# m-dayani/EORB_SLAM

Hardware: AMD Instinct MI355X
Metric: front-end frames/s (event-accumulate + extract + match) per GPU; HBM GB/s vs roofline (higher is better)
Workload: dtype f32; 1 GPU; BASELINE.json configs[1]: synthetic 1000000 events/slice on 240x180 (shapes generator, DAVIS sensor pixels; raw (x,y,t,p) records resolved on the GPU through the calibrator's undistortion maps built from the EvETHZ intrinsics, as the reference loader does on the CPU), ev2im_gauss sigma=1 -> ORB-1000 (1.2, 4 levels, FAST 10/0, edge 19) -> SearchForInitialization vs previous slice; input=raw, sequences_per_gpu=1, parallelism=1 GPU

## Files before the change

### eorb_slam_amd/csrc/ev_common.h

```cpp
#pragma once
#include <hip/hip_runtime.h>
#include <stdint.h>
#include <string.h>
#include <algorithm>
#include <vector>
#include "eorb_ctx.h"

namespace eorb {

struct BinLayout {
    int B, nchunks, NT, nb;
    size_t cd, sc, eb, cnt;
    const ChunkDesc* d_chunks = nullptr; const int* d_slice_c0 = nullptr; const int64_t* d_slice_eb = nullptr;
    uint16_t* d_segcnt = nullptr; uint32_t* d_segbase = nullptr; uint32_t* d_tile_cnt = nullptr; uint32_t* d_tile_base = nullptr;
    BinLayout() : BinLayout(0, 0, 0) {}
    BinLayout(int B_, int nchunks_, int NT_) : B(B_), nchunks(nchunks_), NT(NT_), nb(B_ * NT_)
    {
        cd = sizeof(ChunkDesc) * (size_t)std::max(nchunks, 1);
        sc = (sizeof(int) * (size_t)(B + 1) + 7) & ~(size_t)7;
        eb = sizeof(int64_t) * (size_t)B;
        cnt = (sizeof(uint16_t) * (size_t)std::max(nchunks, 1) * NT + 15) & ~(size_t)15;
    }
    size_t chunks_bytes() const { return cd + sc + eb; }
    size_t segoff_bytes() const { return cnt + sizeof(uint32_t) * (size_t)std::max(nchunks, 1) * NT; }
    void view(void* chunks, void* segoff, void* tile_order)
    {
        d_chunks = (const ChunkDesc*)chunks; d_slice_c0 = (const int*)((char*)chunks + cd); d_slice_eb = (const int64_t*)((char*)chunks + cd + sc);
        d_segcnt = (uint16_t*)segoff; d_segbase = (uint32_t*)((char*)segoff + cnt);
        d_tile_cnt = (uint32_t*)tile_order; d_tile_base = d_tile_cnt + nb;
    }
};

struct EntryBaseRule { int per_event; int64_t slack; int64_t align; };
struct HostBins { std::vector<ChunkDesc> cds; std::vector<int> slice_c0; std::vector<int64_t> slice_eb; int64_t nchunks = 0, entries = 0; };

static inline HostBins bin_chunks_host(const int64_t* h_offsets, int B, int chunk, const EntryBaseRule& R, bool lists = true)
{
    HostBins hb;
    if (lists) { hb.slice_c0.resize(B + 1); hb.slice_eb.resize(B); }
    for (int b = 0; b < B; b++) {
        const int64_t s = h_offsets[b], e = h_offsets[b + 1];
        if (lists) {
            hb.slice_c0[b] = (int)hb.nchunks; hb.slice_eb[b] = hb.entries;
            for (int64_t k = s; k < e; k += chunk) {
                ChunkDesc cd; cd.start = k; cd.n = (int32_t)std::min<int64_t>(chunk, e - k); cd.slice = b;
// ... 63 lines not shown
```

### eorb_slam_amd/csrc/ev_plan.h

```cpp
#pragma once
#include <math.h>
#include <stddef.h>
#include <stdint.h>
#include <algorithm>

namespace eorb {

constexpr int kTile = 8;
constexpr int kChunk = 4096;
constexpr int kScatWaves = 8;
constexpr int kSlotScatWaves = 8;
constexpr int kSlotCountWaves = 16;
constexpr int kHotCap = 8192;
constexpr int kHotRows = 240;
constexpr int kDdLog = 20;
constexpr int kDirectSlices = 8;
constexpr int64_t kDirectMaxEvents = 16384;

struct AccumShape {
    int h;
    int R, dup;
    int TX, TY, NT, NTp;
    int nbits;
    int64_t nev, per_slice;
// ... 90 lines not shown
inline bool plan_sparse_gather(const AccumShape& S, const AccumRequest& Q, const AccumKnobs& K)
{
    return Q.raw && !Q.mode_count && (K.gather_form == 2 || (K.gather_form == 0 && plan_sparse_load(S, Q.B)));
}

enum { kGatherSparse, kGatherRawRows, kGatherGeneric };
struct GatherPlan { int kind, NC, threads, per_wave; };
inline GatherPlan plan_gather(const AccumShape& S, const AccumRequest& Q, const AccumKnobs& K)
{
    const int nb = Q.B * S.NT;
    if (plan_sparse_gather(S, Q, K)) return GatherPlan{kGatherSparse, 0, 0, nb >= 65536 ? 16 : 1};
    if (Q.raw && !Q.mode_count) {
        const int NC = K.gather_nc == 2 || K.gather_nc == 4 ? K.gather_nc : (nb >= 32768 ? 4 : 2);
        return GatherPlan{kGatherRawRows, NC, 64 * (1 + 8 / NC), 0};
    }
    return GatherPlan{kGatherGeneric, 0, K.gather_threads, 0};
}

struct SlotScatterChoice { int chunk, waves; bool rank; size_t lds; };
inline size_t plan_slot_lds_rank(int NT, int chunk, int waves) { const int NTp = (NT + 1) & ~1; return ((size_t)NT * 4 + (size_t)chunk * 4 * 2 + (size_t)waves * NTp * 2 + (size_t)(NTp + 2) * 2 + (size_t)chunk * 4 + 15) & ~(size_t)15; }
inline size_t plan_slot_lds_pre(int NT, int chunk) { const int NTp = (NT + 1) & ~1; return ((size_t)NT * 4 + (size_t)chunk * 4 * 2 + (size_t)(NTp + 2) * 2 + (size_t)chunk * 4 + 15) & ~(size_t)15; }
inline size_t plan_slot_lds_ballot(int NT, int chunk) { const int NTp = (NT + 1) & ~1; return ((size_t)chunk * 4 + (size_t)chunk * 2 + (size_t)chunk * 4 * 2 + (size_t)kSlotScatWaves * NTp * 2 + (size_t)(NTp + 2) * 2 + (size_t)NT * 4 + 15) & ~(size_t)15; }

inline bool plan_slot_scatter(const AccumShape& S, const AccumKnobs& K, bool rank_ok, SlotScatterChoice* out)
{
    const int pref = K.slot_chunk ? K.slot_chunk : (S.per_slice >= (int64_t)1 << 18 ? 4096 : (S.per_slice >= (int64_t)1 << 17 ? 2048 : (S.per_slice >= (int64_t)1 << 14 ? 1024 : 256)));
    const bool rank_allowed = rank_ok && K.slot_rank;
    static const int sizes[4] = {4096, 2048, 1024, 256};
    for (int i = 0; i < 4; i++) {
        const int chunk = sizes[i];
        if (chunk > pref) continue;
        if (rank_allowed) {
            const int waves = chunk == 4096 ? 16 : kSlotScatWaves;
            const size_t l = plan_slot_lds_rank(S.NT, chunk, waves);
            if (l <= (size_t)(chunk == 4096 ? 79 : 158) * 1024) { *out = SlotScatterChoice{chunk, waves, true, l}; return true; }
        }
        if (chunk <= 2048) {
            const size_t l = plan_slot_lds_ballot(S.NT, chunk);
            if (l <= 64 * 1024) { *out = SlotScatterChoice{chunk, kSlotScatWaves, false, l}; return true; }
        }
    }
    return false;
}

inline bool plan_slot_shape(const AccumShape& S, int B, const AccumKnobs& K, bool rank_ok, SlotScatterChoice* out)
{
    return !(B > 2048 || (size_t)S.NT * 4 > 64 * 1024 || !plan_slot_scatter(S, K, rank_ok, out));
}

enum { kCountGlobal, kCountLds, kCountLdsKeyed };
enum { kRecAsIs, kRecShort2, kRecRanked8 };
// ... 73 lines not shown
```

### eorb_slam_amd/csrc/ev_slots.hip

```cpp
#include "eorb_ctx.h"
#include "ev_common.h"
#include "dev_math.h"
#include "sl_hot_asm.h"
#include <algorithm>
#include <stdlib.h>
#include <string.h>
#include <vector>

namespace eorb {

constexpr uint32_t kNoSlot = 0xffu;
typedef uint16_t slot_entry;
constexpr uint32_t kEntryTag = 0x1000u;
constexpr uint16_t kNoGeo = 0xffffu;

__global__ void sl_assign_kernel(const uint32_t* __restrict__ src_info, int nsrc, int W, int H, int h, int TX,
                                 uint32_t* __restrict__ tile_nslots, uint2* __restrict__ slot_tab, uint16_t* __restrict__ slot_geo,
                                 int* __restrict__ info)
{
    const int i = blockIdx.x * blockDim.x + threadIdx.x;
    if (i >= nsrc) { if (i == nsrc) slot_geo[i] = kNoGeo; return; }
    const uint32_t w = src_info[i];
    const int xi = (int)(int16_t)(w & 0xffff), yi = (int)(int16_t)(w >> 16);
    uint2 o = make_uint2(0u, 0xffffffffu);
// ... 106 lines not shown
    }
    if (blockIdx.x == 0) {
        if (tid < B) slice_eb[tid] = e0[tid];
        for (int b = tid; b <= B; b += blockDim.x) slice_c0[b] = c0[b];
    }
    const int g = blockIdx.x * blockDim.x + tid;
    if (g >= nchunks) return;
    int lo = 0, hi = B;
    while (hi - lo > 1) { const int mid = (lo + hi) >> 1; if (c0[mid] <= g) lo = mid; else hi = mid; }
    const int64_t start = off[lo] + ((int64_t)(g - c0[lo]) << chunk_shift);
    ChunkDesc cd; cd.start = start; cd.n = (int32_t)min(chunk, off[lo + 1] - start); cd.slice = lo;
    chunks[g] = cd;
}

template <int stride>
__device__ __forceinline__ uint32_t sl_load_rec(const unsigned char* e, int k)
{
    if (stride == 2) { const uint32_t v = *(const uint16_t*)(e + (size_t)k * 2); return v == 0xffffu ? 0x7fffffffu : v; }
    return *(const uint32_t*)(e + (size_t)k * (size_t)(stride < 0 ? -stride : stride));
}
template <int stride>
__global__ __launch_bounds__(256) void sl_count_kernel(const eorb_raw_event* __restrict__ ev, const ChunkDesc* __restrict__ chunks,
                                                       const uint2* __restrict__ slot_tab, int LW, int LH, int TX, int NT,
                                                       uint16_t* __restrict__ segcnt)
{
    extern __shared__ uint32_t cnt[];
    const ChunkDesc cd = chunks[blockIdx.x];
    for (int i = threadIdx.x; i < NT; i += blockDim.x) cnt[i] = 0;
    __syncthreads();
    const unsigned char* e = (const unsigned char*)ev + (size_t)cd.start * (size_t)(stride < 0 ? -stride : stride);
    const uint32_t xmask = stride == 4 ? 0x7fffu : 0xffffu;
    const bool hashed = stride < 0 || stride == 2;
    constexpr int U = 8;
    for (int k0 = threadIdx.x; k0 < cd.n; k0 += blockDim.x * U) {
        uint32_t xy[U], rg[U];
#pragma unroll
        for (int u = 0; u < U; u++) { const int k = k0 + u * blockDim.x; xy[u] = k < cd.n ? sl_load_rec<stride>(e, k) : 0xffffffffu; }
#pragma unroll
        for (int u = 0; u < U; u++) {
            const int x = (int)(xy[u] & xmask), y = (int)(xy[u] >> 16);
            const uint32_t row = xy[u] & 0x7fffffffu;
            if (hashed) rg[u] = (row != 0x7fffffffu && row < (uint32_t)LW * (uint32_t)LH) ? slot_tab[row].x : 0u;
            else rg[u] = (x < LW && y < LH) ? slot_tab[(uint32_t)y * (uint32_t)LW + x].x : 0u;
        }
#pragma unroll
        for (int u = 0; u < U; u++) {
            const int nx = (rg[u] >> 16) & 3, ny = (rg[u] >> 18) & 3;
            const int t0 = (int)((rg[u] >> 8) & 0xff) * TX + (int)(rg[u] & 0xff);
            if (nx && ny) {
                atomicAdd(&cnt[t0], 1u);
                if (nx > 1) atomicAdd(&cnt[t0 + 1], 1u);
                if (ny > 1) { atomicAdd(&cnt[t0 + TX], 1u); if (nx > 1) atomicAdd(&cnt[t0 + TX + 1], 1u); }
            }
        }
    }
    __syncthreads();
    uint16_t* sc = segcnt + (size_t)blockIdx.x * NT;
    for (int i = threadIdx.x; i < NT; i += blockDim.x) sc[i] = (uint16_t)cnt[i];
}

__device__ __forceinline__ uint32_t sl_dict_hash(uint64_t k)
{
    k ^= k >> 33; k *= 0xff51afd7ed558ccdull; k ^= k >> 33; k *= 0xc4ceb9fe1a85ec53ull; k ^= k >> 33;
    return (uint32_t)k;
}
template <int stride, bool KEYED = false, bool RANKS = false>
__global__ __launch_bounds__(64 * kSlotCountWaves) void sl_count_lds_kernel(const eorb_raw_event* __restrict__ ev, const ChunkDesc* __restrict__ chunks,
                                                                       int nchunks, const uint16_t* __restrict__ slot_geo, int LW, int LH,
                                                                       int TX, int NT, uint16_t* __restrict__ segcnt, SlotDict D = SlotDict{nullptr, 0u, nullptr, nullptr, 0},
                                                                       uint16_t* __restrict__ rec16 = nullptr)
{
    extern __shared__ uint32_t smc[];
    const int tid = threadIdx.x, lane = tid & 63, wave = tid >> 6;
    const int ntab = (LW * LH + 2) >> 1, NTp = (NT + 1) & ~1;
    for (int i = tid; i < ntab; i += 64 * kSlotCountWaves) smc[i] = ((const uint32_t*)slot_geo)[i];
    const uint16_t* tab = (const uint16_t*)smc;
    uint32_t* cnt = smc + ntab + wave * (NTp >> 1);
    __syncthreads();
    constexpr int astride = stride < 0 ? -stride : stride;
    const uint32_t xmask = stride == 4 ? 0x7fffu : 0xffffu;
    constexpr int U = 8;
    for (int ch = blockIdx.x * kSlotCountWaves + wave; ch < nchunks; ch += gridDim.x * kSlotCountWaves) {
        const ChunkDesc cd = chunks[ch];
        for (int i = lane; i < (NTp >> 1); i += 64) cnt[i] = 0u;
        const unsigned char* e = (const unsigned char*)ev + (size_t)cd.start * (size_t)astride;
        uint32_t xyn[U];
        if (!KEYED) {
#pragma unroll
            for (int u = 0; u < U; u++) { const int k = lane + u * 64; xyn[u] = k < cd.n ? sl_load_rec<stride>(e, k) : 0xffffffffu; }
        }
        for (int k0 = lane; k0 < cd.n; k0 += 64 * U) {
            uint32_t xy[U], g[U];
// ... 60 lines not shown
                            }
                        }
                    }
                    const int k = k0 + u * 64;
                    if (k < cd.n) ((uint64_t*)rec16)[cd.start + k] = (uint64_t)(r16[u] & 0xffffu) | (rk << 16);
                }
                continue;
            }
#pragma unroll
            for (int u = 0; u < U; u++) {
                if (g[u] != kNoGeo) {
                    const int t0 = (int)((g[u] >> 7) & 0x7f) * TX + (int)(g[u] & 0x7f);
                    const bool two_x = (g[u] >> 14) & 1, two_y = (g[u] >> 15) & 1;
                    atomicAdd(&cnt[t0 >> 1], 1u << (16 * (t0 & 1)));
                    if (two_x) atomicAdd(&cnt[(t0 + 1) >> 1], 1u << (16 * ((t0 + 1) & 1)));
                    if (two_y) {
                        atomicAdd(&cnt[(t0 + TX) >> 1], 1u << (16 * ((t0 + TX) & 1)));
                        if (two_x) atomicAdd(&cnt[(t0 + TX + 1) >> 1], 1u << (16 * ((t0 + TX + 1) & 1)));
                    }
                }
            }
        }
        __builtin_amdgcn_wave_barrier();
        uint16_t* sc = segcnt + (size_t)ch * NT;
        const uint16_t* c16 = (const uint16_t*)cnt;
        for (int i = lane; i < NT; i += 64) sc[i] = c16[i];
        __builtin_amdgcn_wave_barrier();
    }
}

__global__ __launch_bounds__(1024) void sl_scan_kernel(const int* __restrict__ slice_chunk0, const uint16_t* __restrict__ segcnt, int NT,
                                                       uint32_t* __restrict__ segbase, uint32_t* __restrict__ tile_cnt,
                                                       uint32_t* __restrict__ tile_base)
{
    __shared__ uint32_t wsum[16];
    __shared__ uint32_t carry;
    const int slice = blockIdx.x;
    const int c0 = slice_chunk0[slice], c1 = slice_chunk0[slice + 1];
    const int lane = threadIdx.x & 63, wave = threadIdx.x >> 6;
    if (threadIdx.x == 0) carry = 0;
    __syncthreads();
    for (int t0 = 0; t0 < NT; t0 += blockDim.x) {
        const int tile = t0 + threadIdx.x;
        uint32_t run = 0;
        if (tile < NT) {
            int c = c0;
            for (; c + 8 <= c1; c += 8) {
                uint32_t v[8];
#pragma unroll
                for (int u = 0; u < 8; u++) v[u] = segcnt[(size_t)(c + u) * NT + tile];
#pragma unroll
                for (int u = 0; u < 8; u++) { segbase[(size_t)(c + u) * NT + tile] = run; run += v[u]; }
            }
            for (; c < c1; c++) { const uint32_t v = segcnt[(size_t)c * NT + tile]; segbase[(size_t)c * NT + tile] = run; run += v; }
            tile_cnt[(size_t)slice * NT + tile] = run;
        }
        const uint32_t padded = (run + 15u) & ~15u;
        uint32_t incl = (uint32_t)wave_incl_scan((int)padded);
        if (lane == 63) wsum[wave] = incl;
        __syncthreads();
        uint32_t before = carry;
        for (int w = 0; w < wave; w++) before += wsum[w];
        if (tile < NT) tile_base[(size_t)slice * NT + tile] = before + incl - padded;
        __syncthreads();
        if (threadIdx.x == blockDim.x - 1) carry = before + incl;
        __syncthreads();
    }
}

__global__ __launch_bounds__(64 * kSlotScatWaves) void sl_scatter_kernel(const eorb_raw_event* __restrict__ ev, const ChunkDesc* __restrict__ chunks,
                                                                         const uint2* __restrict__ slot_tab, int stride, int LW, int LH, int TX, int TY,
                                                                         int NT, int chunk_cap, const int64_t* __restrict__ slice_ebase,
                                                                         const uint32_t* __restrict__ segbase, const uint32_t* __restrict__ tile_base,
                                                                         slot_entry* __restrict__ entries)
{
    extern __shared__ unsigned char sm2[];
    __shared__ uint32_t s_wsum[kSlotScatWaves];
    constexpr int NTHR = 64 * kSlotScatWaves;
    constexpr int R = 2;
    const int tid = threadIdx.x, lane = tid & 63, wave = tid >> 6;
    const int chunk = blockIdx.x;
    const ChunkDesc cd = chunks[chunk];
    const int NTp = (NT + 1) & ~1;
    uint32_t* pay = (uint32_t*)sm2;
    uint16_t* prng = (uint16_t*)(pay + chunk_cap);
    uint16_t* sidx = prng + chunk_cap;
    uint16_t* cntw = sidx + (size_t)chunk_cap * R * R;
    uint16_t* loff = cntw + kSlotScatWaves * NTp;
    uint32_t* gbase = (uint32_t*)(loff + NTp + 2);
    for (int i = tid; i < kSlotScatWaves * NTp / 2; i += NTHR) ((uint32_t*)cntw)[i] = 0u;
    const unsigned char* e = (const unsigned char*)ev + (size_t)cd.start * (size_t)(stride < 0 ? -stride : stride);
    const uint32_t xmask = stride == 4 ? 0x7fffu : 0xffffu;
    const bool hashed = stride < 0 || stride == 2;
    const int Q = (((cd.n + kSlotScatWaves - 1) / kSlotScatWaves) + 63) & ~63;
    const int S = Q >> 6;
    constexpr int SMAX = 4;
// ... 24 lines not shown
            prng[k] = (uint16_t)(rg & 0xffff);
            if (nx && ny) {
                rng[s] = rg;
                const int t0 = (int)((rg >> 8) & 0xff) * TX + (int)(rg & 0xff);
                for (int dy = 0; dy < ny; dy++)
                    for (int dx = 0; dx < nx; dx++) {
                        const int t = t0 + dy * TX + dx;
                        atomicAdd(&cw32[t >> 1], 1u << (16 * (t & 1)));
                    }
            }
        }
    }
    __syncthreads();
    {
        const int per = (NT + NTHR - 1) / NTHR;
        const int t0 = tid * per, t1 = min(t0 + per, NT);
        uint32_t mine = 0;
        for (int t = t0; t < t1; t++) {
            uint32_t run = 0;
#pragma unroll
            for (int w = 0; w < kSlotScatWaves; w++) { const uint32_t v = cntw[w * NTp + t]; cntw[w * NTp + t] = (uint16_t)run; run += v; }
            loff[t] = (uint16_t)run;
            mine += run;
            gbase[t] = tile_base[(size_t)cd.slice * NT + t] + segbase[(size_t)chunk * NT + t];
        }
        uint32_t incl = (uint32_t)wave_incl_scan((int)mine);
        if (lane == 63) s_wsum[wave] = incl;
        __syncthreads();
        uint32_t before = incl - mine;
        for (int w = 0; w < wave; w++) before += s_wsum[w];
        for (int t = t0; t < t1; t++) { const uint32_t v = loff[t]; loff[t] = (uint16_t)before; before += v; }
        if (tid == NTHR - 1) loff[NT] = (uint16_t)before;
    }
    __syncthreads();
    const uint64_t lt_mask = (lane == 0) ? 0ull : (~0ull >> (64 - lane));
    uint16_t* cw = cntw + wave * NTp;
    const int txr = (TX + R - 1) / R;
    int mbits = 1; while ((1 << mbits) < txr * ((TY + R - 1) / R)) mbits++;
#pragma unroll
    for (int s = 0; s < SMAX; s++) {
        if (s >= S) break;
        const uint32_t rg = rng[s];
        const int tx0 = rg & 0xff, ty0 = (rg >> 8) & 0xff, tx1 = tx0 + (int)((rg >> 16) & 3) - 1, ty1 = ty0 + (int)((rg >> 18) & 3) - 1;
        const bool valid = rg != 0u;
        const uint16_t kloc = (uint16_t)(wave * Q + s * 64 + lane);
#pragma unroll
        for (int cy = 0; cy < R; cy++) {
// ... 10 lines not shown
                    const bool bit = (mkey >> b) & 1;
                    const uint64_t bal = __ballot(bit);
                    m &= bit ? bal : ~bal;
                }
                if (has) {
                    const int rank = __popcll(m & lt_mask);
                    const uint32_t base = cw[key];
                    sidx[(uint32_t)loff[key] + base + rank] = (uint16_t)(kloc | ((tx - tx0) << 11) | ((ty - ty0) << 13));
                    if (rank == 0) cw[key] = (uint16_t)(base + (uint32_t)__popcll(m));
                }
            }
        }
    }
    __syncthreads();
    slot_entry* out = entries + (size_t)slice_ebase[cd.slice];
    const int E = loff[NT];
    for (int p = tid; p < E; p += NTHR) {
        const uint32_t sv = sidx[p];
        const int k = sv & 0x7ff;
        const int dx = (sv >> 11) & 3, dy = (sv >> 13) & 3;
        const uint32_t r0 = prng[k];
        const int t = ((int)(r0 >> 8) + dy) * TX + (int)(r0 & 0xff) + dx;
        const uint32_t slot = (pay[k] >> (8 * (dy * 2 + dx))) & 0xffu;
        out[(size_t)gbase[t] + (uint32_t)(p - (int)loff[t])] = (slot_entry)(kEntryTag | slot);
    }
}

template <int stride, int NW >
__global__ __launch_bounds__(64 * NW) void sl_scatter_rank_kernel(const eorb_raw_event* __restrict__ ev, const ChunkDesc* __restrict__ chunks,
                                                                              const uint2* __restrict__ slot_tab, int LW, int LH, int TX, int NT,
                                                                              int chunk_cap, const int64_t* __restrict__ slice_ebase,
                                                                              const uint32_t* __restrict__ segbase, const uint32_t* __restrict__ tile_base,
                                                                              slot_entry* __restrict__ entries)
{
    extern __shared__ unsigned char sm2[];
    __shared__ uint32_t s_wsum[NW];
    constexpr int NTHR = 64 * NW;
    const int tid = threadIdx.x, lane = tid & 63, wave = tid >> 6;
    const int chunk = blockIdx.x;
    const ChunkDesc cd = chunks[chunk];
    const int NTp = (NT + 1) & ~1;
    uint32_t* gbase = (uint32_t*)sm2;
    uint16_t* stile = (uint16_t*)(gbase + NT);
    uint16_t* cntw = stile + (size_t)chunk_cap * 4;
    uint16_t* loff = cntw + NW * NTp;
    uint8_t* sorted = (uint8_t*)(loff + NTp + 2);
    for (int i = tid; i < NW * NTp / 2; i += NTHR) ((uint32_t*)cntw)[i] = 0u;
    const unsigned char* e = (const unsigned char*)ev + (size_t)cd.start * (size_t)(stride < 0 ? -stride : stride);
    const uint32_t xmask = stride == 4 ? 0x7fffu : 0xffffu;
    const bool hashed = stride < 0 || stride == 2;
    const int Q = (((cd.n + NW - 1) / NW) + 63) & ~63;
    const int S = Q >> 6;
    constexpr int SMAX = 4;
    __syncthreads();
    uint32_t* cw32 = (uint32_t*)(cntw + wave * NTp);
// ... 32 lines not shown
    }
    __syncthreads();
#if defined(EORB_KO_SCAT) && EORB_KO_SCAT == 1
    if (rk[0] == 0x12345678u) entries[0] = 0; return;
#endif
    {
        const int per = (NT + NTHR - 1) / NTHR;
        const int t0 = tid * per, t1 = min(t0 + per, NT);
        uint32_t mine = 0;
        for (int t = t0; t < t1; t++) {
            uint32_t run = 0;
#pragma unroll
            for (int w = 0; w < NW; w++) { const uint32_t v = cntw[w * NTp + t]; cntw[w * NTp + t] = (uint16_t)run; run += v; }
            loff[t] = (uint16_t)run;
            mine += run;
        }
        uint32_t incl = (uint32_t)wave_incl_scan((int)mine);
        if (lane == 63) s_wsum[wave] = incl;
        __syncthreads();
        uint32_t before = incl - mine;
        for (int w = 0; w < wave; w++) before += s_wsum[w];
        for (int t = t0; t < t1; t++) {
            const uint32_t v = loff[t]; loff[t] = (uint16_t)before;
            gbase[t] = tile_base[(size_t)cd.slice * NT + t] + segbase[(size_t)chunk * NT + t] - before;
            before += v;
        }
        if (tid == NTHR - 1) loff[NT] = (uint16_t)before;
    }
    __syncthreads();
#if defined(EORB_KO_SCAT) && EORB_KO_SCAT == 2
    if (rk[0] == 0x12345678u) entries[0] = 0; return;
#endif
    const uint16_t* cw = cntw + wave * NTp;
#pragma unroll
    for (int s = 0; s < SMAX; s++) {
        const uint32_t rg = rst[s].x, sb = rst[s].y;
        const int nx = (rg >> 16) & 3, ny = (rg >> 18) & 3;
        const int tx0 = rg & 0xff, ty0 = (rg >> 8) & 0xff;
#pragma unroll
        for (int j = 0; j < 4; j++) {
#ifdef EORB_TEST_RANK_ORDER_BUG
            const int dx = j & 1, dy = j >> 1;
#else
            const int dx = ((j & 1) - tx0) & 1, dy = ((j >> 1) - ty0) & 1;
#endif
            if (nx && ny && dx < nx && dy < ny) {
                const int t = (ty0 + dy) * TX + tx0 + dx;
                const uint32_t pos = (uint32_t)loff[t] + cw[t] + ((rk[s] >> (8 * j)) & 0xffu);
                sorted[pos] = (uint8_t)((sb >> (8 * (dy * 2 + dx))) & 0xffu);
                stile[pos] = (uint16_t)t;
            }
        }
    }
    __syncthreads();
#if defined(EORB_KO_SCAT) && EORB_KO_SCAT == 3
    if (rk[0] == 0x12345678u) entries[0] = 0; return;
#endif
    slot_entry* out = entries + (size_t)slice_ebase[cd.slice];
    const int E = loff[NT];
    for (int p = tid; p < E; p += NTHR) out[(size_t)(uint32_t)(gbase[stile[p]] + (uint32_t)p)] = (slot_entry)(kEntryTag | sorted[p]);
}

template <int NW>
__global__ __launch_bounds__(64 * NW) void sl_scatter_pre_kernel(const uint64_t* __restrict__ rec, const ChunkDesc* __restrict__ chunks,
                                                                 const uint2* __restrict__ slot_tab, int nsrc, int TX, int NT, int chunk_cap,
                                                                 const int64_t* __restrict__ slice_ebase, const uint16_t* __restrict__ segcnt,
                                                                 const uint32_t* __restrict__ segbase, const uint32_t* __restrict__ tile_base,
                                                                 slot_entry* __restrict__ entries)
{
    extern __shared__ unsigned char sm2[];
    __shared__ uint32_t s_wsum[NW];
    constexpr int NTHR = 64 * NW;
    const int tid = threadIdx.x, lane = tid & 63, wave = tid >> 6;
    const int chunk = blockIdx.x;
    const ChunkDesc cd = chunks[chunk];
    const int NTp = (NT + 1) & ~1;
    uint32_t* gbase = (uint32_t*)sm2;
    uint16_t* stile = (uint16_t*)(gbase + NT);
    uint16_t* loff = stile + (size_t)chunk_cap * 4;
    uint8_t* sorted = (uint8_t*)(loff + NTp + 2);
    const int Q = (((cd.n + NW - 1) / NW) + 63) & ~63;
    const int S = Q >> 6;
    constexpr int SMAX = 4;
    uint64_t rr[SMAX]; uint2 rst[SMAX];
#pragma unroll
    for (int s = 0; s < SMAX; s++) {
        const int k = wave * Q + s * 64 + lane;
        rr[s] = (s < S && k < cd.n) ? rec[cd.start + k] : 0xffffull;
    }
#pragma unroll
    for (int s = 0; s < SMAX; s++) {
        const uint32_t row = (uint32_t)(rr[s] & 0xffffull);
        rst[s] = (row != 0xffffu && row < (uint32_t)nsrc) ? slot_tab[row] : make_uint2(0u, 0xffffffffu);
    }
    {
        const int per = (NT + NTHR - 1) / NTHR;
        const int t0 = tid * per, t1 = min(t0 + per, NT);
        const uint16_t* sc = segcnt + (size_t)chunk * NT;
        uint32_t mine = 0;
        for (int t = t0; t < t1; t++) mine += sc[t];
        uint32_t incl = (uint32_t)wave_incl_scan((int)mine);
        if (lane == 63) s_wsum[wave] = incl;
        __syncthreads();
        uint32_t before = incl - mine;
        for (int w = 0; w < wave; w++) before += s_wsum[w];
        for (int t = t0; t < t1; t++) {
            const uint32_t v = sc[t];
            loff[t] = (uint16_t)before;
            gbase[t] = tile_base[(size_t)cd.slice * NT + t] + segbase[(size_t)chunk * NT + t] - before;
            before += v;
        }
        if (tid == NTHR - 1) loff[NT] = (uint16_t)before;
    }
    __syncthreads();
#if defined(EORB_KO_SCAT) && EORB_KO_SCAT == 2
    if (rst[0].x == 0x12345678u) entries[0] = 0; return;
#endif
#pragma unroll
    for (int s = 0; s < SMAX; s++) {
        const uint32_t rg = rst[s].x, sb = rst[s].y;
        const int nx = (rg >> 16) & 3, ny = (rg >> 18) & 3;
        const int tx0 = rg & 0xff, ty0 = (rg >> 8) & 0xff;
        const uint64_t rk = rr[s] >> 16;
#pragma unroll
        for (int j = 0; j < 4; j++) {
            const int dx = ((j & 1) - tx0) & 1, dy = ((j >> 1) - ty0) & 1;
            if (nx && ny && dx < nx && dy < ny) {
                const int t = (ty0 + dy) * TX + tx0 + dx;
                const uint32_t pos = (uint32_t)loff[t] + (uint32_t)((rk >> (12 * j)) & 0xfffull);
                sorted[pos] = (uint8_t)((sb >> (8 * (dy * 2 + dx))) & 0xffu);
                stile[pos] = (uint16_t)t;
            }
        }
    }
    __syncthreads();
#if defined(EORB_KO_SCAT) && EORB_KO_SCAT == 3
// ... 482 lines not shown
    size_t plan_bytes() const { return sizeof(uint4) * (size_t)L.nb + sizeof(uint32_t) * ((size_t)gp.Gt + 5 * (size_t)NT); }
    uint4* d_items() const { return (uint4*)ws.plan.p; }
    uint32_t* d_task() const { return (uint32_t*)(d_items() + L.nb); }
    uint32_t* d_tile_m() const { return d_task() + gp.Gt; }
    uint32_t* d_scr() const { return d_tile_m() + NT; }
    uint32_t* d_tile_w() const { return d_scr() + 2 * (size_t)NT; }
    uint32_t* d_ctr() const { return d_tile_w() + NT; }
    uint32_t* d_hot_cnt() const { return (uint32_t*)ws.hot.p; }
    HotDesc* d_hot_items() const { return (HotDesc*)((char*)ws.hot.p + 256); }
    slot_entry* d_entries() const { return (slot_entry*)ws.entries.p; }
};

static int slots_layout(SlotPart& p)
{
    eorb_ctx* c = p.c; eorb_ctx::SlotWS& ws = p.ws;
    const int B = p.B, NT = p.NT, chunk = p.sc.chunk;
    const bool on_dev = B <= kOffsetsInArg;
    const HostBins hb = bin_chunks_host(p.h_offsets, B, chunk, EntryBaseRule{4, (int64_t)NT * 16, 16}, !on_dev);
    if (hb.nchunks >= (int64_t)1 << 31) return set_err(c, EORB_E_CAPACITY, "ev_accumulate: too many chunks");
    p.L = BinLayout(B, (int)hb.nchunks, NT);
    const BinLayout& L = p.L;
    int rc;
    if ((rc = ensure(c, ws.chunks, L.chunks_bytes()))) return rc;
    if ((rc = ensure(c, ws.segoff, L.segoff_bytes()))) return rc;
    if ((rc = ensure(c, ws.entries, sizeof(slot_entry) * (size_t)hb.entries + 8192))) return rc;
    if ((rc = ensure(c, ws.tile_order, sizeof(uint32_t) * 2 * (size_t)L.nb))) return rc;
    if ((rc = ensure(c, ws.plan, p.plan_bytes()))) return rc;
    if ((rc = ensure(c, ws.hot, sizeof(HotDesc) * (size_t)kHotBuckets * kHotCap + 256))) return rc;
    if (p.bp.record != kRecAsIs && (rc = ensure(c, ws.rec16, (p.bp.record == kRecRanked8 ? sizeof(uint64_t) : sizeof(uint16_t)) * (size_t)std::max<int64_t>(p.h_offsets[B], 1)))) return rc;
#ifdef EORB_SLOT_TRACE
    if ((rc = ensure(c, c->sl_trace, sizeof(unsigned long long) * 6 * 16 * (size_t)p.gp.Gt + 64))) return rc;
#endif
    if (on_dev) {
        SliceOffsets so;
        for (int b = 0; b <= B; b++) so.off[b] = p.h_offsets[b];
        sl_chunks_kernel<<<std::max(1, (L.nchunks + 255) / 256), 256, 0, p.M>>>(so, B, chunk == 4096 ? 12 : (chunk == 2048 ? 11 : (chunk == 1024 ? 10 : 8)), NT, L.nchunks, (ChunkDesc*)ws.chunks.p,
                                                                                 (int*)((char*)ws.chunks.p + L.cd), (int64_t*)((char*)ws.chunks.p + L.cd + L.sc));
    }
    else if ((rc = bin_chunks_upload(c, L, hb, ws.chunks.p, p.M))) return rc;
    p.L.view(ws.chunks.p, ws.segoff.p, ws.tile_order.p);
    return EORB_OK;
}

static int slots_count_scan(const SlotPart& p)
{
    eorb_ctx* c = p.c; const PosTables& T = p.T; const BinLayout& L = p.L; const SlotBinPlan& bp = p.bp;
    int rc;
    {
        ProfScope ps(c, "ev_count");
        if (L.nchunks && bp.count == kCountGlobal) {
            const SlCountFn fn = sl_count_fn(bp.stride);
            fn<<<L.nchunks, 256, bp.lds_count, p.M>>>((const eorb_raw_event*)p.d_events, L.d_chunks, p.d_tab(), T.w, T.h, p.TX, p.NT, L.d_segcnt);
        }
        else if (L.nchunks) {
            const SlCountLdsFn fn = sl_count_lds_fn(bp);
            if ((rc = sl_optin(c, (const void*)fn, 159 * 1024))) return rc;
            fn<<<std::min(p.ncu, (L.nchunks + kSlotCountWaves - 1) / kSlotCountWaves), 64 * kSlotCountWaves, bp.lds_count, p.M>>>(
                (const eorb_raw_event*)p.d_events, L.d_chunks, L.nchunks, p.d_geo(), T.w, T.h, p.TX, p.NT, L.d_segcnt,
                p.dict ? *p.dict : SlotDict{nullptr, 0u, nullptr, nullptr, 0}, bp.record != kRecAsIs ? (uint16_t*)p.ws.rec16.p : nullptr);
        }
    }
    ProfScope ps(c, "ev_scan");
    sl_scan_kernel<<<p.B, 1024, 0, p.M>>>(L.d_slice_c0, L.d_segcnt, p.NT, L.d_segbase, L.d_tile_cnt, L.d_tile_base);
    return EORB_OK;
}

static int slots_scatter(const SlotPart& p)
{
    eorb_ctx* c = p.c; const PosTables& T = p.T; const BinLayout& L = p.L; const SlotBinPlan& bp = p.bp;
    const int chunk = p.sc.chunk, waves = p.sc.waves;
    const eorb_raw_event* d_ev = p.dict ? (const eorb_raw_event*)p.dict->rec : (const eorb_raw_event*)(bp.record == kRecShort2 ? p.ws.rec16.p : p.d_events);
    int rc;
    {
        ProfScope ps(c, "ev_scatter");
        if (L.nchunks && bp.scatter == kScatPre) {
            const SlScatPreFn fn = sl_scatter_pre_fn(waves);
            if ((rc = sl_optin(c, (const void*)fn, 159 * 1024))) return rc;
            fn<<<L.nchunks, 64 * waves, bp.lds_scatter, p.M>>>((const uint64_t*)p.ws.rec16.p, L.d_chunks, p.d_tab(), T.w * T.h, p.TX, p.NT, chunk, L.d_slice_eb, L.d_segcnt, L.d_segbase,
                                                               L.d_tile_base, p.d_entries());
        }
        else if (L.nchunks && bp.scatter == kScatRank) {
            const SlScatRankFn fn = sl_scatter_rank_fn(bp.scat_stride, waves);
            if ((rc = sl_optin(c, (const void*)fn, 159 * 1024))) return rc;
            fn<<<L.nchunks, 64 * waves, bp.lds_scatter, p.M>>>(d_ev, L.d_chunks, p.d_tab(), T.w, T.h, p.TX, p.NT, chunk, L.d_slice_eb, L.d_segbase, L.d_tile_base, p.d_entries());
        }
        else if (L.nchunks)
            sl_scatter_kernel<<<L.nchunks, 64 * kSlotScatWaves, bp.lds_scatter, p.M>>>(d_ev, L.d_chunks, p.d_tab(), bp.scat_stride, T.w, T.h, p.TX, p.TY, p.NT, chunk, L.d_slice_eb, L.d_segbase,
                                                                                         L.d_tile_base, p.d_entries());
        EORB_LAUNCH_CHECK(c, "ev_bin (slot) kernels");
    }
    EORB_HIP(c, hipEventRecord(p.E[2], p.M));
    return EORB_OK;
}

static int slots_fork_plan(const SlotPart& p)
{
    eorb_ctx* c = p.c; const BinLayout& L = p.L; const SlotGatherPlan& g = p.gp;
    EORB_HIP(c, hipEventRecord(p.E[0], p.M));
    EORB_HIP(c, hipStreamWaitEvent(p.P, p.E[0], 0));
    EORB_HIP(c, hipMemsetAsync(p.ws.hot.p, 0, 256, p.P));
    sl_plan_kernel<<<p.NT, 256, sizeof(uint32_t) * 2 * (size_t)p.B, p.P>>>(L.d_tile_cnt, L.d_tile_base, L.d_slice_eb, p.B, p.NT, p.TX, g.hot_min, p.d_nslots(), p.d_rowbase(),
                                                                             p.d_items(), p.d_tile_w(), p.d_tile_m(), p.d_ctr(), p.d_hot_cnt(), p.d_hot_items(), g.hot_cap);
    sl_tasks_kernel<<<1, 1024, sizeof(uint32_t) * (size_t)p.NT, p.P>>>(p.d_tile_w(), p.d_tile_m(), p.NT, g.Gt, g.max_per_tile, p.d_scr(), p.d_task(), p.d_hot_cnt(), g.hot_cap);
    EORB_HIP(c, hipEventRecord(p.E[1], p.P));
    return EORB_OK;
}

static int slots_gather(const SlotPart& p)
{
    eorb_ctx* c = p.c; const PosTables& T = p.T; const SlotGatherPlan& g = p.gp;
    int rc;
// ... 70 lines not shown
```

Baseline: 47290 frames/s.

## Store per-chunk exclusive tile offsets and fold tile base into chunk gbase rows

The count kernels now write per-chunk exclusive prefix offsets (loff rows) instead of raw per-tile counts. The scan kernel parallelises over both tiles and chunk segments, each thread handling 8 tiles. It emits one precomputed global base per chunk and tile, with the tile base and local offset already folded in, using vectorised stores. Scatter kernels load these rows directly rather than redoing the per-chunk scan and combining segbase with tile_base, which removes redundant scans and global reads. The cost is a more complex two-pass scan with shared-memory segment totals, plus an implicit 16-bit limit on per-chunk entry counts.

```diff
diff --git a/eorb_slam_amd/csrc/ev_common.h b/eorb_slam_amd/csrc/ev_common.h
--- a/eorb_slam_amd/csrc/ev_common.h
+++ b/eorb_slam_amd/csrc/ev_common.h
@@ -20,7 +20,12 @@
         sc = (sizeof(int) * (size_t)(B + 1) + 7) & ~(size_t)7;
         eb = sizeof(int64_t) * (size_t)B;
         cnt = (sizeof(uint16_t) * (size_t)std::max(nchunks, 1) * NT + 15) & ~(size_t)15;
+        rows = plan_slot_rows(nchunks, NT); lp = rows.lp; gp = rows.gp;
     }
+    int lp = 0, gp = 0; SlotRows rows{0, 0, 0, 0};
+    uint16_t* d_loff = nullptr; uint32_t* d_gbase = nullptr;
+    size_t slot_rows_bytes() const { return rows.bytes; }
+    void view_slot_rows(void* segoff) { d_loff = (uint16_t*)segoff; d_gbase = (uint32_t*)((char*)segoff + rows.loff_bytes); }
     size_t chunks_bytes() const { return cd + sc + eb; }
     size_t segoff_bytes() const { return cnt + sizeof(uint32_t) * (size_t)std::max(nchunks, 1) * NT; }
     void view(void* chunks, void* segoff, void* tile_order)
diff --git a/eorb_slam_amd/csrc/ev_plan.h b/eorb_slam_amd/csrc/ev_plan.h
--- a/eorb_slam_amd/csrc/ev_plan.h
+++ b/eorb_slam_amd/csrc/ev_plan.h
@@ -136,11 +136,29 @@
 inline size_t plan_slot_lds_pre(int NT, int chunk) { const int NTp = (NT + 1) & ~1; return ((size_t)NT * 4 + (size_t)chunk * 4 * 2 + (size_t)(NTp + 2) * 2 + (size_t)chunk * 4 + 15) & ~(size_t)15; }
 inline size_t plan_slot_lds_ballot(int NT, int chunk) { const int NTp = (NT + 1) & ~1; return ((size_t)chunk * 4 + (size_t)chunk * 2 + (size_t)chunk * 4 * 2 + (size_t)kSlotScatWaves * NTp * 2 + (size_t)(NTp + 2) * 2 + (size_t)NT * 4 + 15) & ~(size_t)15; }
 
+constexpr int kSlotChunkMax = 4096;
+static_assert(4 * kSlotChunkMax <= 0xffff, "a chunk's entry count, loff[NT], is a 16-bit word");
+inline int plan_slot_loff_pitch(int NT) { return (NT + 2) & ~1; }
+inline int plan_slot_gbase_pitch(int NT) { return (NT + 3) & ~3; }
+struct SlotRows { int lp, gp; size_t loff_bytes, bytes; };
+inline SlotRows plan_slot_rows(int nchunks, int NT)
+{
+    SlotRows r;
+    const size_t n = (size_t)std::max(nchunks, 1);
+    r.lp = plan_slot_loff_pitch(NT); r.gp = plan_slot_gbase_pitch(NT);
+    r.loff_bytes = (sizeof(uint16_t) * n * r.lp + 15) & ~(size_t)15;
+    r.bytes = r.loff_bytes + sizeof(uint32_t) * n * r.gp;
+    return r;
+}
+constexpr int kSlotScanTiles = 8;
+inline int plan_slot_scan_waves(int NT) { return std::min(16, ((NT + kSlotScanTiles - 1) / kSlotScanTiles + 63) / 64); }
+inline int plan_slot_scan_segments(int NT) { return 16 / plan_slot_scan_waves(NT); }
+
 inline bool plan_slot_scatter(const AccumShape& S, const AccumKnobs& K, bool rank_ok, SlotScatterChoice* out)
 {
     const int pref = K.slot_chunk ? K.slot_chunk : (S.per_slice >= (int64_t)1 << 18 ? 4096 : (S.per_slice >= (int64_t)1 << 17 ? 2048 : (S.per_slice >= (int64_t)1 << 14 ? 1024 : 256)));
     const bool rank_allowed = rank_ok && K.slot_rank;
-    static const int sizes[4] = {4096, 2048, 1024, 256};
+    static const int sizes[4] = {kSlotChunkMax, 2048, 1024, 256};
     for (int i = 0; i < 4; i++) {
         const int chunk = sizes[i];
         if (chunk > pref) continue;
diff --git a/eorb_slam_amd/csrc/ev_slots.hip b/eorb_slam_amd/csrc/ev_slots.hip
--- a/eorb_slam_amd/csrc/ev_slots.hip
+++ b/eorb_slam_amd/csrc/ev_slots.hip
@@ -152,9 +152,10 @@
 template <int stride>
 __global__ __launch_bounds__(256) void sl_count_kernel(const eorb_raw_event* __restrict__ ev, const ChunkDesc* __restrict__ chunks,
                                                        const uint2* __restrict__ slot_tab, int LW, int LH, int TX, int NT,
-                                                       uint16_t* __restrict__ segcnt)
+                                                       int LP, uint16_t* __restrict__ loff)
 {
     extern __shared__ uint32_t cnt[];
+    __shared__ uint32_t s_wsum[4];
     const ChunkDesc cd = chunks[blockIdx.x];
     for (int i = threadIdx.x; i < NT; i += blockDim.x) cnt[i] = 0;
     __syncthreads();
@@ -185,8 +186,21 @@
         }
     }
     __syncthreads();
-    uint16_t* sc = segcnt + (size_t)blockIdx.x * NT;
-    for (int i = threadIdx.x; i < NT; i += blockDim.x) sc[i] = (uint16_t)cnt[i];
+    const int lane = threadIdx.x & 63, wave = threadIdx.x >> 6;
+    const int per = (NT + 255) / 256;
+    const int t0 = min((int)threadIdx.x * per, NT), t1 = min(t0 + per, NT);
+    uint32_t mine = 0;
+    for (int t = t0; t < t1; t++) mine += cnt[t];
+    const uint32_t incl = (uint32_t)wave_incl_scan((int)mine);
+    if (lane == 63) s_wsum[wave] = incl;
+    __syncthreads();
+    uint32_t before = incl - mine;
+    for (int w = 0; w < wave; w++) before += s_wsum[w];
+    for (int t = t0; t < t1; t++) { const uint32_t v = cnt[t]; cnt[t] = before; before += v; }
+    __syncthreads();
+    uint16_t* lo = loff + (size_t)blockIdx.x * LP;
+    for (int i = threadIdx.x; i < NT; i += 256) lo[i] = (uint16_t)cnt[i];
+    if (threadIdx.x == 255) { lo[NT] = (uint16_t)before; if (NT + 1 < LP) lo[NT + 1] = 0; }
 }
 
 __device__ __forceinline__ uint32_t sl_dict_hash(uint64_t k)
@@ -197,7 +211,7 @@
 template <int stride, bool KEYED = false, bool RANKS = false>
 __global__ __launch_bounds__(64 * kSlotCountWaves) void sl_count_lds_kernel(const eorb_raw_event* __restrict__ ev, const ChunkDesc* __restrict__ chunks,
                                                                        int nchunks, const uint16_t* __restrict__ slot_geo, int LW, int LH,
-                                                                       int TX, int NT, uint16_t* __restrict__ segcnt, SlotDict D = SlotDict{nullptr, 0u, nullptr, nullptr, 0},
+                                                                       int TX, int NT, int LP, uint16_t* __restrict__ loff, SlotDict D = SlotDict{nullptr, 0u, nullptr, nullptr, 0},
                                                                        uint16_t* __restrict__ rec16 = nullptr)
 {
     extern __shared__ uint32_t smc[];
@@ -304,48 +318,116 @@
             }
         }
         __builtin_amdgcn_wave_barrier();
-        uint16_t* sc = segcnt + (size_t)ch * NT;
-        const uint16_t* c16 = (const uint16_t*)cnt;
-        for (int i = lane; i < NT; i += 64) sc[i] = c16[i];
+        const int nd = NTp >> 1, per = (nd + 63) >> 6;
+        const int d0 = min(lane * per, nd), d1 = min(d0 + per, nd);
+        uint32_t mine = 0;
+        for (int d = d0; d < d1; d++) { const uint32_t w = cnt[d]; mine += (w & 0xffffu) + (w >> 16); }
+        const uint32_t incl = (uint32_t)wave_incl_scan((int)mine);
+        uint32_t before = incl - mine;
+        for (int d = d0; d < d1; d++) { const uint32_t w = cnt[d]; const uint32_t lo = before; before += w & 0xffffu; cnt[d] = lo | (before << 16); before += w >> 16; }
         __builtin_amdgcn_wave_barrier();
-    }
-}
-
-__global__ __launch_bounds__(1024) void sl_scan_kernel(const int* __restrict__ slice_chunk0, const uint16_t* __restrict__ segcnt, int NT,
-                                                       uint32_t* __restrict__ segbase, uint32_t* __restrict__ tile_cnt,
+        uint32_t* so = (uint32_t*)(loff + (size_t)ch * LP);
+        for (int i = lane; i < nd; i += 64) so[i] = cnt[i];
+        if (!(NT & 1) && lane == 63) so[nd] = incl;
+        __builtin_amdgcn_wave_barrier();
+    }
+}
+
+__global__ __launch_bounds__(1024) void sl_scan_kernel(const int* __restrict__ slice_chunk0, const uint16_t* __restrict__ loff, int NT, int LP, int GP,
+                                                       uint32_t* __restrict__ gbase, uint32_t* __restrict__ tile_cnt,
                                                        uint32_t* __restrict__ tile_base)
 {
+    constexpr int T = kSlotScanTiles, ND = T / 2 + 1, U1 = 8, U2 = 4;
+    __shared__ uint32_t segtot[16 * 64 * T];
     __shared__ uint32_t wsum[16];
-    __shared__ uint32_t carry;
     const int slice = blockIdx.x;
     const int c0 = slice_chunk0[slice], c1 = slice_chunk0[slice + 1];
-    const int lane = threadIdx.x & 63, wave = threadIdx.x >> 6;
-    if (threadIdx.x == 0) carry = 0;
-    __syncthreads();
-    for (int t0 = 0; t0 < NT; t0 += blockDim.x) {
-        const int tile = t0 + threadIdx.x;
-        uint32_t run = 0;
-        if (tile < NT) {
-            int c = c0;
-            for (; c + 8 <= c1; c += 8) {
-                uint32_t v[8];
-#pragma unroll
-                for (int u = 0; u < 8; u++) v[u] = segcnt[(size_t)(c + u) * NT + tile];
-#pragma unroll
-                for (int u = 0; u < 8; u++) { segbase[(size_t)(c + u) * NT + tile] = run; run += v[u]; }
-            }
-            for (; c < c1; c++) { const uint32_t v = segcnt[(size_t)c * NT + tile]; segbase[(size_t)c * NT + tile] = run; run += v; }
-            tile_cnt[(size_t)slice * NT + tile] = run;
-        }
-        const uint32_t padded = (run + 15u) & ~15u;
-        uint32_t incl = (uint32_t)wave_incl_scan((int)padded);
+    const int lane = threadIdx.x & 63, wave = __builtin_amdgcn_readfirstlane((int)(threadIdx.x >> 6));
+    const int NG = (NT + T - 1) / T;
+    const int GW = min(16, (NG + 63) >> 6), GT = GW * 64;
+    const int NS = 16 / GW;
+    const int seg = wave / GW, gl = (wave - seg * GW) * 64 + lane;
+    const bool act = seg < NS;
+    const int nper = (c1 - c0 + NS - 1) / NS;
+    const int cs = act ? min(c0 + seg * nper, c1) : c1, ce = min(cs + nper, c1);
+    const int LPd = LP >> 1;
+    auto load_row = [&](int c, int t0, uint32_t (&w)[ND]) {
+        const uint32_t* row = (const uint32_t*)(loff + (size_t)c * LP);
+#pragma unroll
+        for (int k = 0; k < ND; k++) w[k] = row[min((t0 >> 1) + k, LPd - 1)];
+    };
+    auto half = [](const uint32_t (&w)[ND], int j) { return (w[j >> 1] >> (16 * (j & 1))) & 0xffffu; };
+    uint32_t carry = 0;
+    for (int g0 = 0; g0 < NG; g0 += GT) {
+        const int t0 = (g0 + gl) * T;
+        const bool mine = act && t0 < NT;
+        uint32_t tot[T];
+#pragma unroll
+        for (int j = 0; j < T; j++) tot[j] = 0u;
+        if (mine)
+            for (int c = cs; c < ce; c += U1) {
+                uint32_t w[U1][ND];
+#pragma unroll
+                for (int u = 0; u < U1; u++) {
+                    if (c + u < ce) load_row(c + u, t0, w[u]);
+                    else {
+#pragma unroll
+                        for (int k = 0; k < ND; k++) w[u][k] = 0u;
+                    }
+                }
+#pragma unroll
+                for (int u = 0; u < U1; u++)
+#pragma unroll
+                    for (int j = 0; j < T; j++) tot[j] += t0 + j < NT ? half(w[u], j + 1) - half(w[u], j) : 0u;
+            }
+        if (act) {
+#pragma unroll
+            for (int j = 0; j < T; j++) segtot[(seg * T + j) * GT + gl] = tot[j];
+        }
+        __syncthreads();
+        uint32_t run[T], padsum = 0u;
+#pragma unroll
+        for (int j = 0; j < T; j++) {
+            uint32_t before = 0u, all = 0u;
+            if (act)
+                for (int s = 0; s < NS; s++) { const uint32_t v = segtot[(s * T + j) * GT + gl]; before += s < seg ? v : 0u; all += v; }
+            run[j] = before; tot[j] = all; padsum += (all + 15u) & ~15u;
+        }
+        const uint32_t incl = (uint32_t)wave_incl_scan((int)padsum);
         if (lane == 63) wsum[wave] = incl;
         __syncthreads();
-        uint32_t before = carry;
-        for (int w = 0; w < wave; w++) before += wsum[w];
-        if (tile < NT) tile_base[(size_t)slice * NT + tile] = before + incl - padded;
-        __syncthreads();
-        if (threadIdx.x == blockDim.x - 1) carry = before + incl;
+        uint32_t tb = carry + incl - padsum;
+        for (int w = seg * GW; w < wave; w++) tb += wsum[w];
+        for (int w = 0; w < GW; w++) carry += wsum[w];
+        if (mine) {
+#pragma unroll
+            for (int j = 0; j < T; j++) {
+                if (seg == 0 && t0 + j < NT) { tile_cnt[(size_t)slice * NT + t0 + j] = tot[j]; tile_base[(size_t)slice * NT + t0 + j] = tb; }
+                run[j] += tb; tb += (tot[j] + 15u) & ~15u;
+            }
+            for (int c = cs; c < ce; c += U2) {
+                uint32_t w[U2][ND];
+#pragma unroll
+                for (int u = 0; u < U2; u++) {
+                    if (c + u < ce) load_row(c + u, t0, w[u]);
+                    else {
+#pragma unroll
+                        for (int k = 0; k < ND; k++) w[u][k] = 0u;
+                    }
+                }
+#pragma unroll
+                for (int u = 0; u < U2; u++) {
+                    uint32_t o[T];
+#pragma unroll
+                    for (int j = 0; j < T; j++) { const uint32_t l = half(w[u], j); o[j] = run[j] - l; run[j] += t0 + j < NT ? half(w[u], j + 1) - l : 0u; }
+                    if (c + u < ce) {
+                        uint4* dst = (uint4*)(gbase + (size_t)(c + u) * GP + t0);
+#pragma unroll
+                        for (int q = 0; q < T / 4; q++) if (t0 + 4 * q < NT) dst[q] = make_uint4(o[4 * q], o[4 * q + 1], o[4 * q + 2], o[4 * q + 3]);
+                    }
+                }
+            }
+        }
         __syncthreads();
     }
 }
@@ -353,7 +435,7 @@
 __global__ __launch_bounds__(64 * kSlotScatWaves) void sl_scatter_kernel(const eorb_raw_event* __restrict__ ev, const ChunkDesc* __restrict__ chunks,
                                                                          const uint2* __restrict__ slot_tab, int stride, int LW, int LH, int TX, int TY,
                                                                          int NT, int chunk_cap, const int64_t* __restrict__ slice_ebase,
-                                                                         const uint32_t* __restrict__ segbase, const uint32_t* __restrict__ tile_base,
+                                                                         const uint32_t* __restrict__ gbase_rows, int GP,
                                                                          slot_entry* __restrict__ entries)
 {
     extern __shared__ unsigned char sm2[];
@@ -424,7 +506,7 @@
             for (int w = 0; w < kSlotScatWaves; w++) { const uint32_t v = cntw[w * NTp + t]; cntw[w * NTp + t] = (uint16_t)run; run += v; }
             loff[t] = (uint16_t)run;
             mine += run;
-            gbase[t] = tile_base[(size_t)cd.slice * NT + t] + segbase[(size_t)chunk * NT + t];
+            gbase[t] = gbase_rows[(size_t)chunk * GP + t];
         }
         uint32_t incl = (uint32_t)wave_incl_scan((int)mine);
         if (lane == 63) s_wsum[wave] = incl;
@@ -481,7 +563,7 @@
         const uint32_t r0 = prng[k];
         const int t = ((int)(r0 >> 8) + dy) * TX + (int)(r0 & 0xff) + dx;
         const uint32_t slot = (pay[k] >> (8 * (dy * 2 + dx))) & 0xffu;
-        out[(size_t)gbase[t] + (uint32_t)(p - (int)loff[t])] = (slot_entry)(kEntryTag | slot);
+        out[(size_t)(uint32_t)(gbase[t] + (uint32_t)p)] = (slot_entry)(kEntryTag | slot);
     }
 }
 
@@ -489,7 +571,7 @@
 __global__ __launch_bounds__(64 * NW) void sl_scatter_rank_kernel(const eorb_raw_event* __restrict__ ev, const ChunkDesc* __restrict__ chunks,
                                                                               const uint2* __restrict__ slot_tab, int LW, int LH, int TX, int NT,
                                                                               int chunk_cap, const int64_t* __restrict__ slice_ebase,
-                                                                              const uint32_t* __restrict__ segbase, const uint32_t* __restrict__ tile_base,
+                                                                              const uint32_t* __restrict__ gbase_rows, int GP,
                                                                               slot_entry* __restrict__ entries)
 {
     extern __shared__ unsigned char sm2[];
@@ -568,7 +650,7 @@
         for (int w = 0; w < wave; w++) before += s_wsum[w];
         for (int t = t0; t < t1; t++) {
             const uint32_t v = loff[t]; loff[t] = (uint16_t)before;
-            gbase[t] = tile_base[(size_t)cd.slice * NT + t] + segbase[(size_t)chunk * NT + t] - before;
+            gbase[t] = gbase_rows[(size_t)chunk * GP + t];
             before += v;
         }
         if (tid == NTHR - 1) loff[NT] = (uint16_t)before;
@@ -610,12 +692,11 @@
 template <int NW>
 __global__ __launch_bounds__(64 * NW) void sl_scatter_pre_kernel(const uint64_t* __restrict__ rec, const ChunkDesc* __restrict__ chunks,
                                                                  const uint2* __restrict__ slot_tab, int nsrc, int TX, int NT, int chunk_cap,
-                                                                 const int64_t* __restrict__ slice_ebase, const uint16_t* __restrict__ segcnt,
-                                                                 const uint32_t* __restrict__ segbase, const uint32_t* __restrict__ tile_base,
+                                                                 const int64_t* __restrict__ slice_ebase, const uint16_t* __restrict__ loff_rows, int LP,
+                                                                 const uint32_t* __restrict__ gbase_rows, int GP,
                                                                  slot_entry* __restrict__ entries)
 {
     extern __shared__ unsigned char sm2[];
-    __shared__ uint32_t s_wsum[NW];
     constexpr int NTHR = 64 * NW;
     const int tid = threadIdx.x, lane = tid & 63, wave = tid >> 6;
     const int chunk = blockIdx.x;
@@ -634,30 +715,23 @@
         const int k = wave * Q + s * 64 + lane;
         rr[s] = (s < S && k < cd.n) ? rec[cd.start + k] : 0xffffull;
     }
+    const uint32_t* lrow = (const uint32_t*)(loff_rows + (size_t)chunk * LP);
+    const uint32_t* grow = gbase_rows + (size_t)chunk * GP;
+    uint32_t* loff32 = (uint32_t*)loff;
+    const int LPd = LP >> 1;
+    const uint32_t l0 = tid < LPd ? lrow[tid] : 0u, g0 = tid < NT ? grow[tid] : 0u;
 #pragma unroll
     for (int s = 0; s < SMAX; s++) {
         const uint32_t row = (uint32_t)(rr[s] & 0xffffull);
         rst[s] = (row != 0xffffu && row < (uint32_t)nsrc) ? slot_tab[row] : make_uint2(0u, 0xffffffffu);
     }
-    {
-        const int per = (NT + NTHR - 1) / NTHR;
-        const int t0 = tid * per, t1 = min(t0 + per, NT);
-        const uint16_t* sc = segcnt + (size_t)chunk * NT;
-        uint32_t mine = 0;
-        for (int t = t0; t < t1; t++) mine += sc[t];
-        uint32_t incl = (uint32_t)wave_incl_scan((int)mine);
-        if (lane == 63) s_wsum[wave] = incl;
-        __syncthreads();
-        uint32_t before = incl - mine;
-        for (int w = 0; w < wave; w++) before += s_wsum[w];
-        for (int t = t0; t < t1; t++) {
-            const uint32_t v = sc[t];
-            loff[t] = (uint16_t)before;
-            gbase[t] = tile_base[(size_t)cd.slice * NT + t] + segbase[(size_t)chunk * NT + t] - before;
-            before += v;
-        }
-        if (tid == NTHR - 1) loff[NT] = (uint16_t)before;
-    }
+#if defined(EORB_KO_SCAT) && EORB_KO_SCAT == 1
+    if (rst[0].x == 0x12345678u || l0 + g0 == 0x12345678u) entries[0] = 0; return;
+#endif
+    if (tid < LPd) loff32[tid] = l0;
+    if (tid < NT) gbase[tid] = g0;
+    for (int i = tid + NTHR; i < LPd; i += NTHR) loff32[i] = lrow[i];
+    for (int i = tid + NTHR; i < NT; i += NTHR) gbase[i] = grow[i];
     __syncthreads();
 #if defined(EORB_KO_SCAT) && EORB_KO_SCAT == 2
     if (rst[0].x == 0x12345678u) entries[0] = 0; return;
@@ -1186,7 +1260,7 @@
     const BinLayout& L = p.L;
     int rc;
     if ((rc = ensure(c, ws.chunks, L.chunks_bytes()))) return rc;
-    if ((rc = ensure(c, ws.segoff, L.segoff_bytes()))) return rc;
+    if ((rc = ensure(c, ws.segoff, L.slot_rows_bytes()))) return rc;
     if ((rc = ensure(c, ws.entries, sizeof(slot_entry) * (size_t)hb.entries + 8192))) return rc;
     if ((rc = ensure(c, ws.tile_order, sizeof(uint32_t) * 2 * (size_t)L.nb))) return rc;
     if ((rc = ensure(c, ws.plan, p.plan_bytes()))) return rc;
@@ -1203,6 +1277,7 @@
     }
     else if ((rc = bin_chunks_upload(c, L, hb, ws.chunks.p, p.M))) return rc;
     p.L.view(ws.chunks.p, ws.segoff.p, ws.tile_order.p);
+    p.L.view_slot_rows(ws.segoff.p);
     return EORB_OK;
 }
 
@@ -1214,18 +1289,18 @@
         ProfScope ps(c, "ev_count");
         if (L.nchunks && bp.count == kCountGlobal) {
             const SlCountFn fn = sl_count_fn(bp.stride);
-            fn<<<L.nchunks, 256, bp.lds_count, p.M>>>((const eorb_raw_event*)p.d_events, L.d_chunks, p.d_tab(), T.w, T.h, p.TX, p.NT, L.d_segcnt);
+            fn<<<L.nchunks, 256, bp.lds_count, p.M>>>((const eorb_raw_event*)p.d_events, L.d_chunks, p.d_tab(), T.w, T.h, p.TX, p.NT, L.lp, L.d_loff);
         }
         else if (L.nchunks) {
             const SlCountLdsFn fn = sl_count_lds_fn(bp);
             if ((rc = sl_optin(c, (const void*)fn, 159 * 1024))) return rc;
             fn<<<std::min(p.ncu, (L.nchunks + kSlotCountWaves - 1) / kSlotCountWaves), 64 * kSlotCountWaves, bp.lds_count, p.M>>>(
-                (const eorb_raw_event*)p.d_events, L.d_chunks, L.nchunks, p.d_geo(), T.w, T.h, p.TX, p.NT, L.d_segcnt,
+                (const eorb_raw_event*)p.d_events, L.d_chunks, L.nchunks, p.d_geo(), T.w, T.h, p.TX, p.NT, L.lp, L.d_loff,
                 p.dict ? *p.dict : SlotDict{nullptr, 0u, nullptr, nullptr, 0}, bp.record != kRecAsIs ? (uint16_t*)p.ws.rec16.p : nullptr);
         }
     }
     ProfScope ps(c, "ev_scan");
-    sl_scan_kernel<<<p.B, 1024, 0, p.M>>>(L.d_slice_c0, L.d_segcnt, p.NT, L.d_segbase, L.d_tile_cnt, L.d_tile_base);
+    sl_scan_kernel<<<p.B, 1024, 0, p.M>>>(L.d_slice_c0, L.d_loff, p.NT, L.lp, L.gp, L.d_gbase, L.d_tile_cnt, L.d_tile_base);
     return EORB_OK;
 }
 
@@ -1240,17 +1315,17 @@
         if (L.nchunks && bp.scatter == kScatPre) {
             const SlScatPreFn fn = sl_scatter_pre_fn(waves);
             if ((rc = sl_optin(c, (const void*)fn, 159 * 1024))) return rc;
-            fn<<<L.nchunks, 64 * waves, bp.lds_scatter, p.M>>>((const uint64_t*)p.ws.rec16.p, L.d_chunks, p.d_tab(), T.w * T.h, p.TX, p.NT, chunk, L.d_slice_eb, L.d_segcnt, L.d_segbase,
-                                                               L.d_tile_base, p.d_entries());
+            fn<<<L.nchunks, 64 * waves, bp.lds_scatter, p.M>>>((const uint64_t*)p.ws.rec16.p, L.d_chunks, p.d_tab(), T.w * T.h, p.TX, p.NT, chunk, L.d_slice_eb, L.d_loff, L.lp,
+                                                               L.d_gbase, L.gp, p.d_entries());
         }
         else if (L.nchunks && bp.scatter == kScatRank) {
             const SlScatRankFn fn = sl_scatter_rank_fn(bp.scat_stride, waves);
             if ((rc = sl_optin(c, (const void*)fn, 159 * 1024))) return rc;
-            fn<<<L.nchunks, 64 * waves, bp.lds_scatter, p.M>>>(d_ev, L.d_chunks, p.d_tab(), T.w, T.h, p.TX, p.NT, chunk, L.d_slice_eb, L.d_segbase, L.d_tile_base, p.d_entries());
+            fn<<<L.nchunks, 64 * waves, bp.lds_scatter, p.M>>>(d_ev, L.d_chunks, p.d_tab(), T.w, T.h, p.TX, p.NT, chunk, L.d_slice_eb, L.d_gbase, L.gp, p.d_entries());
         }
         else if (L.nchunks)
-            sl_scatter_kernel<<<L.nchunks, 64 * kSlotScatWaves, bp.lds_scatter, p.M>>>(d_ev, L.d_chunks, p.d_tab(), bp.scat_stride, T.w, T.h, p.TX, p.TY, p.NT, chunk, L.d_slice_eb, L.d_segbase,
-                                                                                         L.d_tile_base, p.d_entries());
+            sl_scatter_kernel<<<L.nchunks, 64 * kSlotScatWaves, bp.lds_scatter, p.M>>>(d_ev, L.d_chunks, p.d_tab(), bp.scat_stride, T.w, T.h, p.TX, p.TY, p.NT, chunk, L.d_slice_eb, L.d_gbase,
+                                                                                         L.gp, p.d_entries());
         EORB_LAUNCH_CHECK(c, "ev_bin (slot) kernels");
     }
     EORB_HIP(c, hipEventRecord(p.E[2], p.M));
```

After: 49130 frames/s (median of 6 runs). 1.04x the previous value.
